# ha7ilm/csdr

Measured on AMD Instinct MI355X. Metric: complex MS/s in->out, WFM demod chain @2.4 MS/s x N streams, higher is better.
Workload: dtype f32

## Files before the change

### csdr_amd/csrc/wfm_mfma.hip

```cpp
#include "common.hpp"
#include "wfm_mfma.hpp"
#include <hip/hip_ext.h>
#include <math.h>
#include <string.h>
#include <stdlib.h>
#include <complex>
#include <vector>
using namespace csdr_amd;

namespace csdr_amd {

bool wfm_mfma_supported(int D, int L, int F)
{
    if ((D * F) & 1) return false;
    const int win_off = (18 * D) & ~15;
    const int span_bytes = 2 * (D * (3 * F + 10) + L) - win_off;
    if (span_bytes > 64 * WFM_NK) return false;
    if (D + L + 3 * D * F + 8 > WFM_HIST) return false;
    return true;
}

void wfm_mfma_build_table(int D, int L, int F, float shift_rate, const float *taps, WfmMfmaTable &t)
{
    t.D = D; t.L = L; t.F = F;
// ... 21 lines not shown
            const int q = r / 4, which = (r % 4) / 2, comp = r % 2;
            const long off = (long)D * (F * q + 9 + which) - base_off_samples;
            for (int tp = 0; tp < L; tp++) {
                const long ts = off + tp;
                const std::complex<double> G = a * (double)taps[tp] * std::polar(pow(mag, (double)ts), ang * (double)ts);
                for (int c = 0; c < 2; c++) {
                    const double val = comp == 0 ? (c == 0 ? G.real() : -G.imag()) : (c == 0 ? G.imag() : G.real());
                    const long colb = 2 * ts + c;
                    const int ks = (int)(colb / 64), b = (int)(colb % 64);
                    long qv = lrint(val * qs);
                    const int w2 = (int)(((qv + 128) % 256 + 256) % 256) - 128; qv = (qv - w2) / 256;
                    const int w1 = (int)(((qv + 128) % 256 + 256) % 256) - 128; qv = (qv - w1) / 256;
                    const int dig[3] = {(int)qv, w1, w2};
                    for (int l = 0; l < 3; l++) t.seq_frags[((size_t)(ks * 3 + l) * 64 + (16 * (b / 16) + r)) * 16 + b % 16] = (int8_t)dig[l];
                    gsum[(size_t)(colb / 16) * 16 + r] += val;
                }
            }
        }
        t.seq_cum.assign((size_t)(ngr + 1) * 16, 0.f);
        for (int r = 0; r < 16; r++) {
            double run = 0;
            for (int g = 0; g <= ngr; g++) { t.seq_cum[(size_t)g * 16 + r] = (float)(0.5 * run); if (g < ngr) run += gsum[(size_t)g * 16 + r]; }
        }
    }
}

}

namespace {

typedef int v4i __attribute__((ext_vector_type(4)));

__device__ __forceinline__ float combine_digits(int a0, int a1, int a2)
{
    return fmaf((float)a0, 65536.0f, fmaf((float)a1, 256.0f, (float)a2));
}

__device__ __forceinline__ void tile_rows(const v4i (&acc)[3], const v4i (&snap)[3], bool two, float scale, const float (&k0)[4], const float (&k1)[4],
                                          float2 C0, float2 C1, float &pI, float &pQ, float &cI, float &cQ)
{
    float u0[4];
    if (two) {
        float u1[4];
#pragma unroll
        for (int r = 0; r < 4; r++) {
            u0[r] = fmaf(combine_digits(snap[0][r], snap[1][r], snap[2][r]), scale, k0[r]);
            u1[r] = fmaf(combine_digits(acc[0][r] - snap[0][r], acc[1][r] - snap[1][r], acc[2][r] - snap[2][r]), scale, k1[r]);
        }
        pI = C0.x * u0[0] - C0.y * u0[1] + (C1.x * u1[0] - C1.y * u1[1]); pQ = C0.x * u0[1] + C0.y * u0[0] + (C1.x * u1[1] + C1.y * u1[0]);
        cI = C0.x * u0[2] - C0.y * u0[3] + (C1.x * u1[2] - C1.y * u1[3]); cQ = C0.x * u0[3] + C0.y * u0[2] + (C1.x * u1[3] + C1.y * u1[2]);
    } else {
#pragma unroll
        for (int r = 0; r < 4; r++) u0[r] = fmaf(combine_digits(acc[0][r], acc[1][r], acc[2][r]), scale, k0[r]);
        pI = C0.x * u0[0] - C0.y * u0[1]; pQ = C0.x * u0[1] + C0.y * u0[0];
        cI = C0.x * u0[2] - C0.y * u0[3]; cQ = C0.x * u0[3] + C0.y * u0[2];
    }
}

template <int N> __device__ __forceinline__ void wait_vmcnt() { asm volatile("s_waitcnt vmcnt(%0)" :: "n"(N) : "memory"); }

template <int KB>
__device__ __forceinline__ void wfm_chain(const v4i (&A)[WFM_NK * 3], const v4i (&Bf)[WFM_NK], bool lo_lane, v4i (&acc)[3], v4i (&snap)[3])
{
    const v4i z = {0, 0, 0, 0};
#pragma unroll
    for (int ks = 0; ks < WFM_NK; ks++) {
        if (ks == KB) {
            const v4i lo = lo_lane ? Bf[ks] : z, hi = lo_lane ? z : Bf[ks];
#pragma unroll
            for (int l = 0; l < 3; l++) acc[l] = __builtin_amdgcn_mfma_i32_16x16x64_i8(A[ks * 3 + l], lo, acc[l], 0, 0, 0);
#pragma unroll
            for (int l = 0; l < 3; l++) snap[l] = acc[l];
#pragma unroll
            for (int l = 0; l < 3; l++) acc[l] = __builtin_amdgcn_mfma_i32_16x16x64_i8(A[ks * 3 + l], hi, acc[l], 0, 0, 0);
        } else {
#pragma unroll
            for (int l = 0; l < 3; l++) acc[l] = __builtin_amdgcn_mfma_i32_16x16x64_i8(A[ks * 3 + l], Bf[ks], acc[l], 0, 0, 0);
        }
    }
}

struct SeqParams {
    int n_streams; long long B2; long long tile_first; int n_tiles, tiles_per_seg;
    int stride, win_off; float scale;
    long long two_T;
    float alpha; const float *last_in; float *last_out; int16_t *s16; float *af; size_t out_pitch; long long j_first; int n_audio;
    const uint8_t *head_in; uint8_t *head_out;
    long long col_bytes; int col_chunks, col_audio, n_cols;
    size_t frag_stride, tab_pitch; int tab_len;
    const float *scales;
    const float *lead_d; const int *lead_n; int lead_stride;
};

#ifndef SEQ_RB_KIB
#define SEQ_RB_KIB 9
#endif
constexpr int SEQ_RB = 1024 * SEQ_RB_KIB;
#ifndef SEQ_RING_PAD
#define SEQ_RING_PAD 32
#endif
constexpr int SEQ_RP = SEQ_RB + SEQ_RING_PAD;
constexpr int SEQ_NGR = 4 * WFM_NK;
#ifndef SEQ_TPG_N
#define SEQ_TPG_N 6
#endif
#ifndef SEQ_NLD_N
#define SEQ_NLD_N 2
#endif
constexpr int SEQ_TPG = SEQ_TPG_N;
constexpr int SEQ_NLD = SEQ_NLD_N;
constexpr int SEQ_NW = SEQ_TPG + SEQ_NLD;
constexpr int SEQ_NLW = SEQ_NLD;
constexpr int SEQ_LINE = 64;
constexpr int SEQ_OUTS = (SEQ_LINE - 1 + 3 * 4 * SEQ_TPG + 4 * SEQ_TPG - 1) / (4 * SEQ_TPG);
constexpr int SEQ_OUTR = SEQ_OUTS * 4 * SEQ_TPG;
constexpr int SEQ_OUTP = SEQ_OUTR + 4;
static_assert(16 % SEQ_NLW == 0 && (16 / SEQ_NLW) * 7 <= 63 && SEQ_TPG % 2 == 0, "rows per fetching wave (vmcnt counts to 63); the de-emphasis scan works on pairs");
constexpr int SEQ_HEAD = 1024;

#ifndef WFM_DIAG
#define WFM_DIAG 0
#endif
#ifdef WFM_PROF
__device__ unsigned long long g_wfm_prof[SEQ_NW][8];
__device__ unsigned long long g_wfm_life[SEQ_NW][4];
#define PROF_T(k) { const long long t_now = __builtin_readcyclecounter(); prof[k] += t_now - t_prev; t_prev = t_now; }
#else
#define PROF_T(k)
#endif

constexpr int RES_WARM = 48;
struct ResCtl {
    const uint32_t *desc;
    const uint32_t *ctrl;
    uint32_t *done;
    unsigned *cnt;
    unsigned long long *t_first;
    unsigned long long *next_item;
    unsigned *exiting;
    const uint8_t *in_ring; int16_t *out_ring; size_t in_slot_bytes, out_slot_elems;
    int n_slots, desc_lines, n_wsb, T, D, L, F;
    long long idle_ticks, life_ticks;
    const float *lead_d; int lead_stride;
    const float *lead_state;
    unsigned long long *stats;
    int fence_mode;
};
__device__ __forceinline__ uint32_t sys_load(const uint32_t *p) { return __hip_atomic_load(p, __ATOMIC_RELAXED, __HIP_MEMORY_SCOPE_SYSTEM); }
__device__ __forceinline__ uint32_t res_tag(long long k) { return (uint32_t)((unsigned long long)k % 0xfffffffeull) + 1u; }

template <bool PS, bool RES = false>
__global__ __launch_bounds__(64 * SEQ_NW) void k_wfm_mfma_seq(const uint8_t *__restrict__ in, size_t in_pitch, const v4i *__restrict__ frags, const float *__restrict__ cum,
                                                               const float2 *__restrict__ dtab, const float2 *__restrict__ ctab, SeqParams p_in, ResCtl rc)
{
    static_assert(!(PS && RES), "the resident form exists for the shared-rate kernel");
    constexpr int TPG = SEQ_TPG, SPW = 16 / SEQ_NLW, NTHR = 64 * SEQ_NW;
    extern __shared__ float4 lds_raw[];
    uint8_t *lds_in = reinterpret_cast<uint8_t *>(lds_raw);
    float *lds_out = reinterpret_cast<float *>(lds_in + 16 * SEQ_RP);
    float *lcum = lds_out + 16 * SEQ_OUTP;
    float2 *ctl = reinterpret_cast<float2 *>(lcum + (SEQ_NGR + 1) * 16);
    const int tid = threadIdx.x, wv = __builtin_amdgcn_readfirstlane(tid >> 6), lane = tid & 63, col = lane & 15, q = lane >> 4;
    const bool fetches = wv >= TPG;
#ifdef WFM_PROF
    const long long t_entry = __builtin_readcyclecounter();
    long long t_first = t_entry, t_last = t_entry;
#endif
    const int fw = wv - TPG;
    float scale = p_in.scale;
    if constexpr (PS) { const int sbp = blockIdx.x; frags += (size_t)sbp * p_in.frag_stride; cum += (size_t)sbp * ((SEQ_NGR + 1) * 16); dtab += (size_t)sbp * 3072; ctab += sbp; scale = p_in.scales[sbp]; }
    for (int i = tid; i < (SEQ_NGR + 1) * 16; i += NTHR) lcum[i] = cum[i];
    v4i A[WFM_NK * 3];
#pragma unroll
    for (int s = 0; s < WFM_NK * 3; s++) A[s] = frags[s * 64 + lane];

    float c_lo[4], c_hi[4];
    {
        const float4 a = *reinterpret_cast<const float4 *>(cum + 4 * q), b = *reinterpret_cast<const float4 *>(cum + (size_t)SEQ_NGR * 16 + 4 * q);
        c_lo[0] = a.x; c_lo[1] = a.y; c_lo[2] = a.z; c_lo[3] = a.w; c_hi[0] = b.x; c_hi[1] = b.y; c_hi[2] = b.z; c_hi[3] = b.w;
    }
    const float K = 0.340447550238101026565118445432744920253753662109375f;
    SeqParams p_res;
    if constexpr (RES) p_res = p_in;
    const SeqParams &p = RES ? p_res : p_in;
    unsigned long long item = 0;
    long long res_t_launch = 0;
    uint32_t *const rctl = reinterpret_cast<uint32_t *>(ctl);
    const float2 *const lseed = ctl + 1;
    long long st_wait = 0, st_body = 0, st_done = 0, st_items = 0, st_t = 0;
    if constexpr (RES) { item = rc.next_item[blockIdx.x]; res_t_launch = wall_clock64(); st_t = res_t_launch; }
    bool pend = false; unsigned pend_c = 0; int pend_slot = 0, pend_n = 0; long long pend_k = 0;
    uint32_t pre_v[4] = {0u, 0u, 0u, 0u}; bool pre_valid = false;
    auto res_complete = [&]() {
        if constexpr (RES) {
            if (tid == 0 && pend) {
                pend = false;
                if (pend_c + 1 == (unsigned)rc.n_wsb) {
                    const unsigned long long tf = __hip_atomic_exchange(rc.t_first + pend_slot, ~0ull, __ATOMIC_RELAXED, __HIP_MEMORY_SCOPE_AGENT), td = (unsigned long long)wall_clock64();
                    __hip_atomic_store(rc.cnt + pend_slot, 0u, __ATOMIC_RELAXED, __HIP_MEMORY_SCOPE_AGENT);
                    uint32_t *dn = rc.done + (size_t)pend_slot * 16;
                    __hip_atomic_store(dn + 1, (uint32_t)pend_n, __ATOMIC_RELAXED, __HIP_MEMORY_SCOPE_SYSTEM);
                    __hip_atomic_store(dn + 2, (uint32_t)tf, __ATOMIC_RELAXED, __HIP_MEMORY_SCOPE_SYSTEM); __hip_atomic_store(dn + 3, (uint32_t)(tf >> 32), __ATOMIC_RELAXED, __HIP_MEMORY_SCOPE_SYSTEM);
                    __hip_atomic_store(dn + 4, (uint32_t)td, __ATOMIC_RELAXED, __HIP_MEMORY_SCOPE_SYSTEM); __hip_atomic_store(dn + 5, (uint32_t)(td >> 32), __ATOMIC_RELAXED, __HIP_MEMORY_SCOPE_SYSTEM);
                    asm volatile("s_waitcnt vmcnt(0)" ::: "memory");
                    __hip_atomic_store(dn, res_tag(pend_k), __ATOMIC_RELAXED, __HIP_MEMORY_SCOPE_SYSTEM);
                }
            }
        }
    };
    for (;;) {
    int res_slot = 0, res_lead = 0; long long res_k = 0; bool res_retuned = false;
    const uint8_t *pblock = nullptr;
    if constexpr (RES) {
        res_k = (long long)(item / (unsigned)rc.n_wsb);
        res_slot = (int)(res_k % rc.n_slots);
        if (wv == 0) {
            const uint32_t *dsc = rc.desc + (size_t)res_slot * rc.desc_lines * 16;
            const uint32_t tag = res_tag(res_k);
            const int nd = rc.desc_lines * 16;
            const long long t_wait = wall_clock64();
            uint32_t state = 0;
            for (int iter = 0;; iter++) {
                uint32_t v[4] = {0u, 0u, 0u, 0u};
                bool have = false;
                if (iter == 0 && pre_valid) {
#pragma unroll
                    for (int j = 0; j < 4; j++) v[j] = pre_v[j];
                    have = true;
                } else {
                    const uint32_t t0 = sys_load(dsc);
                    if (t0 == tag) {
#pragma unroll
                        for (int j = 0; j < 4; j++) { const int d = lane + 64 * j; v[j] = d < nd ? sys_load(dsc + d) : 0u; }
                        have = true;
                    }
                }
                const uint32_t ex = __hip_atomic_load(rc.exiting, __ATOMIC_RELAXED, __HIP_MEMORY_SCOPE_AGENT);
                const uint32_t stop = (iter & 7) == 7 ? sys_load(rc.ctrl) : 0u;
                res_complete();
                bool ok = have;
#pragma unroll
                for (int j = 0; j < 4; j++) { const int d = lane + 64 * j; if (d < nd && (d & 15) == 0 && v[j] != tag) ok = false; }
                const bool ready = __all(ok);
                const long long now = wall_clock64();
                const bool old = now - res_t_launch > rc.life_ticks;
                if (ready && !ex && !old) {
#pragma unroll
                    for (int j = 0; j < 4; j++) {
                        const int d = lane + 64 * j, w = d & 15;
                        if (d < nd && w >= 2) rctl[2 + (d >> 4) * 14 + (w - 2)] = v[j];
                        if (d == 1) rctl[1] = v[j];
                    }
                    state = 1; break;
                }
                if (ex || old || stop || now - t_wait > rc.idle_ticks) { state = 2; break; }
                if (iter < 2) __builtin_amdgcn_s_sleep(24); else if (iter < 6) __builtin_amdgcn_s_sleep(64); else { __builtin_amdgcn_s_sleep(127); __builtin_amdgcn_s_sleep(100); }
            }
            pre_valid = false;
            if (lane == 0) rctl[0] = state;
        }
        __syncthreads();
        if (rctl[0] != 1u) {
            if (tid == 0) {
                __hip_atomic_store(rc.exiting, 1u, __ATOMIC_RELAXED, __HIP_MEMORY_SCOPE_AGENT); rc.next_item[blockIdx.x] = item;
                unsigned long long *sp = rc.stats + (size_t)blockIdx.x * 4;
                sp[0] += (unsigned long long)st_wait; sp[1] += (unsigned long long)st_body; sp[2] += (unsigned long long)st_done; sp[3] += (unsigned long long)st_items;
            }
            return;
        }
        if (tid == 0) { const long long t = wall_clock64(); st_wait += t - st_t; st_t = t; }
        res_lead = (int)(rctl[1] & 0xffu); res_retuned = (rctl[1] >> 8) & 1u;
        auto j_hi = [&](long long kk) -> long long {
            if (kk < 0) return -1;
            const long long avail_last = (kk + 1) * rc.T - 1;
            if (avail_last - (rc.L - 1) < 0) return -1;
            const long long k_max = (avail_last - (rc.L - 1)) / rc.D;
            return k_max >= 10 ? (k_max - 10) / rc.F : -1;
        };
        const long long jp = j_hi(res_k - 1), jn = j_hi(res_k);
        p_res.B2 = 2 * res_k * rc.T;
        p_res.j_first = jp + 1; p_res.n_audio = (int)(jn - jp);
        p_res.tile_first = p_res.j_first / 4; p_res.n_tiles = (int)((p_res.j_first + p_res.n_audio - 1) / 4 - p_res.tile_first + 1);
        p_res.tiles_per_seg = p_res.n_tiles;
        p_res.s16 = rc.out_ring + (size_t)res_slot * rc.out_slot_elems;
        if (tid == 0) (void)__hip_atomic_fetch_min(rc.t_first + res_slot, (unsigned long long)wall_clock64(), __ATOMIC_RELAXED, __HIP_MEMORY_SCOPE_AGENT);
    }
    const int sb = RES ? (int)(item % (unsigned)rc.n_wsb) : (int)blockIdx.x;
    const int seg_y = RES ? 0 : (int)blockIdx.y;
    const int col0 = PS ? 16 * seg_y : 0;
    if constexpr (RES) {
        in = rc.in_ring + (size_t)res_slot * rc.in_slot_bytes;
        pblock = rc.in_ring + (size_t)((res_slot + rc.n_slots - 1) % rc.n_slots) * rc.in_slot_bytes + (long long)sb * 16 * (long long)in_pitch;
    }
    const long long t0 = p.tile_first + (long long)seg_y * p.tiles_per_seg * (PS ? 16 : 1);
    long long t1 = t0 + p.tiles_per_seg; if (t1 > p.tile_first + p.n_tiles) t1 = p.tile_first + p.n_tiles;
    if (!RES && t0 >= t1) return;
    const int n_it = (int)(t1 - t0), n_grp = (n_it + TPG - 1) / TPG;
    const int n_lead = RES ? res_lead : ((PS && p.lead_n && seg_y == 0) ? p.lead_n[sb] : 0);
    const int n_warm = RES ? ((res_k > 0 && !res_retuned) ? 2 : 0) : ((PS || seg_y > 0) ? 2 : 0);
    const int last_stream = p.n_streams - 1;
    const int tstride = p.stride;
    const long long org = PS ? (long long)col0 * p.col_bytes : 0LL;
    long long wg = (t0 - (long long)n_warm * TPG) * tstride + p.win_off - p.B2 - org;
    const long long F0 = wg & ~1023LL;
    long long F_end = ((t1 - 1) * tstride + p.win_off - p.B2 - org + 64 * WFM_NK + 1023) & ~1023LL;
    { const long long row_end = ((p.two_T + 1023) & ~1023LL) - org; if (F_end > row_end) F_end = row_end; }
    long long F = F0;
    int fslot = (int)((F0 + 2 * SEQ_RB) % SEQ_RB), wslot = (int)((wg + 2 * SEQ_RB) % SEQ_RB);
    const uint32_t lds_in_addr = (uint32_t)(size_t)(__attribute__((address_space(3))) uint8_t *)lds_in;
    uint32_t voff[SPW], voff_h[SPW];
    long long row_lim[SPW];
#pragma unroll
    for (int r = 0; r < SPW; r++) {
        if constexpr (PS) {
            voff[r] = (uint32_t)((long long)(SPW * fw + r) * p.col_bytes) + 16u * lane;
            voff_h[r] = 16u * lane;
            row_lim[r] = p.two_T - (long long)(col0 + SPW * fw + r) * p.col_bytes;
        } else {
            const int srow = max(min(sb * 16 + SPW * fw + r, last_stream) - sb * 16, 0);
            voff[r] = (uint32_t)srow * (uint32_t)in_pitch + 16u * lane;
            voff_h[r] = (uint32_t)srow * (uint32_t)SEQ_HEAD + 16u * lane;
            row_lim[r] = 0;
        }
    }
    const uint8_t *sblock = PS ? in + (long long)sb * (long long)in_pitch + org : in + (long long)sb * 16 * (long long)in_pitch;
    const uint8_t *hblock = PS ? p.head_in + (size_t)sb * SEQ_HEAD : p.head_in + (size_t)sb * 16 * SEQ_HEAD;
    const bool ragged = (p.two_T & 1023) != 0;
    auto row_step = [&]() {
        if constexpr (PS) {
            const uint32_t ldst = lds_in_addr + (SPW * fw) * SEQ_RP + (uint32_t)fslot;
            const bool head = F < 0 && col0 == 0;
            if (!head && !ragged) {
                uint32_t vo[SPW];
#pragma unroll
                for (int r = 0; r < SPW; r++) vo[r] = F < row_lim[r] ? voff[r] : 16u * lane;
                dma_rows<SPW, SEQ_RP>(vo, sblock + F, __builtin_amdgcn_readfirstlane((int)ldst));
            } else
#pragma unroll
            for (int r = 0; r < SPW; r++) {
                const bool hrow = head && (SPW * fw + r == 0 || F + 1024 > row_lim[r]);
                const bool beyond = !hrow && F >= row_lim[r];
                const uint8_t *sbase = hrow ? hblock : sblock + F;
                const uint32_t vo = hrow ? voff_h[r] : (beyond ? 16u * lane : voff[r]);
                const bool live = hrow || F + 16 * lane < (beyond ? p.two_T - org : row_lim[r]);
                const uint32_t la = __builtin_amdgcn_readfirstlane((int)(ldst + r * SEQ_RP));
                uint32_t keep;
                if (live)
                    asm volatile("s_mov_b32 %0, m0\n\ts_mov_b32 m0, %3\n\ts_nop 0\n\tglobal_load_lds_dwordx4 %1, %2 nt\n\ts_mov_b32 m0, %0"
                                 : "=&s"(keep) : "v"(vo), "s"(sbase), "s"(la) : "memory");
            }
            F += 1024; fslot += 1024; if (fslot >= SEQ_RB) fslot -= SEQ_RB;
            return;
        }
        if constexpr (RES) {
            const uint8_t *sb_res = F < 0 ? pblock + (p.two_T + F) : sblock + F;
            dma_rows<SPW, SEQ_RP>(voff, sb_res, __builtin_amdgcn_readfirstlane((int)(lds_in_addr + (SPW * fw) * SEQ_RP + (uint32_t)fslot)));
            F += 1024; fslot += 1024; if (fslot >= SEQ_RB) fslot -= SEQ_RB;
            return;
        }
        const bool head = F < 0;
        const uint8_t *sbase = head ? hblock : sblock + F;
        const uint32_t ldst = lds_in_addr + (SPW * fw) * SEQ_RP + (uint32_t)fslot;
        const bool mask = ragged && !head;
        const bool live = !mask || F + 16 * lane < p.two_T;
        if (!head && !ragged) dma_rows<SPW, SEQ_RP>(voff, sbase, __builtin_amdgcn_readfirstlane((int)ldst));
        else
#pragma unroll
        for (int r = 0; r < SPW; r++) {
            const uint32_t la = __builtin_amdgcn_readfirstlane((int)(ldst + r * SEQ_RP));
            const uint32_t vo = head ? voff_h[r] : voff[r];
            uint32_t keep;
            if (!mask)
                asm volatile("s_mov_b32 %0, m0\n\ts_mov_b32 m0, %3\n\ts_nop 0\n\tglobal_load_lds_dwordx4 %1, %2 nt\n\ts_mov_b32 m0, %0"
                             : "=&s"(keep) : "v"(vo), "s"(sbase), "s"(la) : "memory");
            else if (live)
                asm volatile("s_mov_b32 %0, m0\n\ts_mov_b32 m0, %3\n\ts_nop 0\n\tglobal_load_lds_dwordx4 %1, %2 nt\n\ts_mov_b32 m0, %0"
                             : "=&s"(keep) : "v"(vo), "s"(sbase), "s"(la) : "memory");
        }
// ... 395 lines not shown
    const int s = blockIdx.x, t = threadIdx.x;
    for (int k = 2 * t; k < 2 * t + 2; k++) {
        const long long pos = two_T - 512 + k;
        head_out[(size_t)s * SEQ_HEAD + 512 + k] = pos >= 0 ? in[(size_t)s * in_pitch + pos] : head_in[(size_t)s * SEQ_HEAD + 512 + (pos + 512)];
    }
}

struct LeadParams { int D, L, F; long long B, j_first, c_first; int n_lead, ja0, lead_stride; float *warm; size_t tab_pitch, dtab_stride, ct_stride, head_pitch, head_off; };
__global__ __launch_bounds__(128) void k_wfm_lead(const uint8_t *__restrict__ in, size_t in_pitch, const uint8_t *__restrict__ head, const float *__restrict__ taps,
                                                 const float2 *__restrict__ ctab, const float2 *__restrict__ dtab, const float2 *__restrict__ dtab_old,
                                                 const int *__restrict__ list, float *__restrict__ lead_d, LeadParams p)
{
    __shared__ float2 yv[2];
    const int s = list[blockIdx.y], ja = (int)blockIdx.x + p.ja0, which = threadIdx.x >> 6, lane = threadIdx.x & 63;
    const long long j = p.j_first + ja, k = (long long)p.F * j + 9 + which;
    const uint8_t *row = in + (size_t)s * in_pitch, *hrow = head + (size_t)s * p.head_pitch + p.head_off;
    const float2 *ct = ctab + (size_t)s * p.ct_stride, *dn = dtab + (size_t)s * p.dtab_stride, *dold = dtab_old + (size_t)s * p.dtab_stride;
    float ai = 0.f, aq = 0.f;
    for (int t = lane; t < p.L; t += 64) {
        const long long n = (long long)p.D * k + t, rel = n - p.B;
        uint32_t vi, vq;
        if (rel < 0) { vi = hrow[2 * (rel + 256)]; vq = hrow[2 * (rel + 256) + 1]; } else { vi = row[2 * rel]; vq = row[2 * rel + 1]; }
        const float2 C = ct[(size_t)((n >> 10) - p.c_first) * p.tab_pitch], Dv = (rel < 0 ? dold : dn)[(int)(n & 1023) + 2048];
        const float2 R = make_float2(C.x * Dv.x - C.y * Dv.y, C.x * Dv.y + C.y * Dv.x);
        const float xi = fmaf((float)vi, 0x1.010102p-7f, -1.0f), xq = fmaf((float)vq, 0x1.010102p-7f, -1.0f);
        const float h = taps[t];
        ai = fmaf(h, xi * R.x - xq * R.y, ai); aq = fmaf(h, xq * R.x + xi * R.y, aq);
    }
#pragma unroll
    for (int o = 32; o >= 1; o >>= 1) { ai += __shfl_xor(ai, o, 64); aq += __shfl_xor(aq, o, 64); }
    if (lane == 0) yv[which] = make_float2(ai, aq);
    __syncthreads();
    if (threadIdx.x == 0) {
        const float K = 0.340447550238101026565118445432744920253753662109375f;
        const float pI = yv[0].x, pQ = yv[0].y, cI = yv[1].x, cQ = yv[1].y;
        const float dq = cQ - pQ, di = cI - pI, num = cI * dq - cQ * di, den = cI * cI + cQ * cQ;
        float rd = __builtin_amdgcn_rcpf(den); rd = fmaf(fmaf(-den, rd, 1.0f), rd, rd);
        const float dv = (den != 0.f) ? (K * num) * rd : 0.f;
        if (ja >= 0) lead_d[(size_t)s * p.lead_stride + ja] = dv; else p.warm[(size_t)s * RES_WARM + (ja + RES_WARM)] = dv;
    }
}

__global__ __launch_bounds__(64) void k_wfm_lead_state(const float *__restrict__ warm, float *__restrict__ state, int n_streams, float alpha)
{
    const int s = blockIdx.x * 64 + threadIdx.x;
    if (s >= n_streams) return;
    float y = 0.f;
    for (int i = 0; i < RES_WARM; i++) y = alpha * warm[(size_t)s * RES_WARM + i] + (1 - alpha) * y;
    state[s] = y;
}

}

namespace csdr_amd {

size_t wfm_mfma_head_bytes(int n_streams) { return (size_t)((n_streams + 15) / 16 * 16) * SEQ_HEAD; }

int wfm_mfma_lead(hipStream_t st, const uint8_t *in, size_t in_pitch, const uint8_t *head, const float *d_taps, const float2 *ctab, size_t tab_pitch, const float2 *d_dtab,
                  const float2 *d_dtab_old, const int *d_list, int n_list, float *d_lead_d, int lead_stride, int D, int L, int F, long long B, long long j_first, int n_lead)
{
    if (n_list <= 0 || n_lead <= 0) return 0;
    LeadParams lp; lp.D = D; lp.L = L; lp.F = F; lp.B = B; lp.j_first = j_first; lp.n_lead = n_lead; lp.tab_pitch = tab_pitch; lp.dtab_stride = 3072;
    lp.ct_stride = 1; lp.head_pitch = SEQ_HEAD; lp.head_off = 512; lp.c_first = (B >> 10) - 1; lp.ja0 = 0; lp.warm = nullptr; lp.lead_stride = lead_stride;
    hipLaunchKernelGGL(k_wfm_lead, dim3(n_lead, n_list), dim3(128), 0, st, in, in_pitch, head, d_taps, ctab, d_dtab, d_dtab_old, d_list, d_lead_d, lp);
    CSDR_LAUNCH_CHECK();
    return 0;
}

int wfm_mfma_lead_shared(hipStream_t st, const uint8_t *in, size_t in_pitch, const uint8_t *prev, size_t two_T, const float *d_taps, const float2 *ctab, const float2 *d_dtab,
                         const float2 *d_dtab_old, const int *d_list, int n_list, float *d_lead_d, int lead_stride, float *d_warm, float *d_state, float alpha,
                         int D, int L, int F, long long B, long long j_first, int n_lead)
{
    if (n_list <= 0) return 0;
    if (j_first < RES_WARM) return fail_msg(-3, "wfm ring: a retune needs %d audio samples in front of the block", RES_WARM);
    LeadParams lp; lp.D = D; lp.L = L; lp.F = F; lp.B = B; lp.j_first = j_first; lp.n_lead = n_lead; lp.tab_pitch = 1; lp.dtab_stride = 0;
    lp.ct_stride = 0; lp.head_pitch = in_pitch; lp.head_off = two_T - 512; lp.c_first = (B >> 10) - 4; lp.ja0 = -RES_WARM; lp.warm = d_warm; lp.lead_stride = lead_stride;
    hipLaunchKernelGGL(k_wfm_lead, dim3(n_lead + RES_WARM, n_list), dim3(128), 0, st, in, in_pitch, prev, d_taps, ctab, d_dtab, d_dtab_old, d_list, d_lead_d, lp);
    CSDR_LAUNCH_CHECK();
    hipLaunchKernelGGL(k_wfm_lead_state, dim3((n_list + 63) / 64), dim3(64), 0, st, d_warm, d_state, n_list, alpha);
    CSDR_LAUNCH_CHECK();
    return 0;
}

int wfm_mfma_launch(hipStream_t st, hipEvent_t ev_begin, hipEvent_t ev_end, const uint8_t *in, size_t in_pitch, const WfmMfmaDevice &dev, const float2 *ctab,
                    int n_streams, int T, long long B, long long j_first, int n_audio, const WfmBackArgs &back, const WfmPerStream *ps)
{
    if (in_pitch * 16 + 4096 >= ((size_t)1 << 32)) return fail_msg(-3, "wfm: in_pitch %zu too large for the matrix-core front end (32-bit row offsets)", in_pitch);
    if (n_audio <= 0) {
        hipLaunchKernelGGL(k_wfm_roll_head, dim3(n_streams), dim3(256), 0, st, in, in_pitch, 2LL * T, back.head_in, back.head_out);
        CSDR_LAUNCH_CHECK();
        return 0;
    }
    SeqParams sp;
    memset((void *)&sp, 0, sizeof sp);
    ResCtl no_res; memset((void *)&no_res, 0, sizeof no_res);
    sp.n_streams = n_streams; sp.B2 = 2 * B; sp.two_T = 2LL * T;
    sp.tile_first = j_first / 4; sp.n_tiles = (int)((j_first + n_audio - 1) / 4 - sp.tile_first + 1);
    sp.stride = dev.tile_stride_bytes; sp.win_off = dev.win_off_bytes; sp.scale = dev.seq_scale;
    const int n_cu = current_device_cu_count();
    const int n_wsb = (n_streams + 15) / 16;
    int n_seg = (n_cu + n_wsb - 1) / n_wsb; if (n_seg < 1) n_seg = 1;
    if (n_seg > sp.n_tiles / 24) n_seg = sp.n_tiles / 24;
    if (n_seg < 1) n_seg = 1;
    sp.tiles_per_seg = ((sp.n_tiles + n_seg - 1) / n_seg + SEQ_TPG - 1) / SEQ_TPG * SEQ_TPG;
    n_seg = (sp.n_tiles + sp.tiles_per_seg - 1) / sp.tiles_per_seg;
    sp.alpha = back.alpha; sp.last_in = back.last_in; sp.last_out = back.last_out; sp.s16 = back.s16; sp.af = back.af; sp.out_pitch = back.out_pitch;
    sp.j_first = j_first; sp.n_audio = n_audio; sp.head_in = back.head_in; sp.head_out = back.head_out;
    if (ps) {
        const long long ts = sp.stride / 2;
        long long per = ts; { long long a = per, b = 1024; while (b) { const long long t = a % b; a = b; b = t; } per = per / a * 1024; }
        int tpp = (int)(per / ts);
        while ((4 * tpp) % SEQ_LINE) tpp *= 2;
        const int n_per = (sp.n_tiles + tpp - 1) / tpp;
        int n_ss = (4 * n_cu + n_streams - 1) / n_streams; if (n_ss < 1) n_ss = 1;
        int np = (n_per + 16 * n_ss - 1) / (16 * n_ss); if (np < 1) np = 1;
        sp.tiles_per_seg = np * tpp;
        sp.n_cols = (sp.n_tiles + sp.tiles_per_seg - 1) / sp.tiles_per_seg;
        n_seg = (sp.n_cols + 15) / 16;
        sp.col_bytes = (long long)sp.tiles_per_seg * sp.stride; sp.col_chunks = (int)(sp.col_bytes / 2048); sp.col_audio = 4 * sp.tiles_per_seg;
        sp.frag_stride = (size_t)WFM_NK * 3 * 64; sp.tab_pitch = ps->tab_pitch; sp.tab_len = ps->tab_len; sp.scales = ps->d_scales;
        sp.lead_d = ps->d_lead_d; sp.lead_n = ps->d_lead_n; sp.lead_stride = ps->lead_stride;
        if (sp.col_bytes * 16 + 4096 >= (1LL << 32)) return fail_msg(-3, "wfm: block too large for the per-stream kernel's 32-bit row offsets");
        const size_t ldsp = (size_t)16 * SEQ_RP + 16 * SEQ_OUTP * sizeof(float) + (SEQ_NGR + 1) * 16 * sizeof(float) + 2 * 48 * sizeof(float2);
        { const int arc = lds_attr_once((const void *)k_wfm_mfma_seq<true>, ldsp); if (arc) return arc; }
        if (ev_begin && ev_end)
            hipExtLaunchKernelGGL(k_wfm_mfma_seq<true>, dim3(n_streams, n_seg), dim3(64 * SEQ_NW), ldsp, st, ev_begin, ev_end, 0, in, in_pitch, (const v4i *)dev.d_seq_frags, dev.d_seq_cum, dev.d_dtab, ctab, sp, no_res);
        else
            hipLaunchKernelGGL(k_wfm_mfma_seq<true>, dim3(n_streams, n_seg), dim3(64 * SEQ_NW), ldsp, st, in, in_pitch, (const v4i *)dev.d_seq_frags, dev.d_seq_cum, dev.d_dtab, ctab, sp, no_res);
        CSDR_LAUNCH_CHECK();
        if (T < 256 || (T & 7)) {
            hipLaunchKernelGGL(k_wfm_roll_head, dim3(n_streams), dim3(256), 0, st, in, in_pitch, 2LL * T, back.head_in, back.head_out);
            CSDR_LAUNCH_CHECK();
        }
        return 0;
    }
    const size_t lds = (size_t)16 * SEQ_RP + 16 * SEQ_OUTP * sizeof(float) + (SEQ_NGR + 1) * 16 * sizeof(float);
    { const int arc = lds_attr_once((const void *)k_wfm_mfma_seq<false>, lds); if (arc) return arc; }
    if (ev_begin && ev_end)
        hipExtLaunchKernelGGL(k_wfm_mfma_seq<false>, dim3(n_wsb, n_seg), dim3(64 * SEQ_NW), lds, st, ev_begin, ev_end, 0, in, in_pitch, (const v4i *)dev.d_seq_frags, dev.d_seq_cum, dev.d_dtab, ctab, sp, no_res);
    else
        hipLaunchKernelGGL(k_wfm_mfma_seq<false>, dim3(n_wsb, n_seg), dim3(64 * SEQ_NW), lds, st, in, in_pitch, (const v4i *)dev.d_seq_frags, dev.d_seq_cum, dev.d_dtab, ctab, sp, no_res);
    CSDR_LAUNCH_CHECK();
    if (T < 256 || (T & 7)) {
        hipLaunchKernelGGL(k_wfm_roll_head, dim3(n_streams), dim3(256), 0, st, in, in_pitch, 2LL * T, back.head_in, back.head_out);
        CSDR_LAUNCH_CHECK();
    }
    return 0;
}

int wfm_mfma_launch_resident(hipStream_t st, hipEvent_t ev_end, const WfmMfmaDevice &dev, int n_streams, size_t in_pitch, float alpha, size_t out_pitch, const WfmResident &rv, int grid)
{
    if (in_pitch * 16 + 4096 >= ((size_t)1 << 32)) return fail_msg(-3, "wfm ring: in_pitch %zu too large (32-bit row offsets)", in_pitch);
    SeqParams sp; memset((void *)&sp, 0, sizeof sp);
    sp.n_streams = n_streams; sp.two_T = 2LL * rv.T; sp.stride = dev.tile_stride_bytes; sp.win_off = dev.win_off_bytes; sp.scale = dev.seq_scale;
    sp.alpha = alpha; sp.out_pitch = out_pitch;
    ResCtl rc; memset((void *)&rc, 0, sizeof rc);
    rc.desc = rv.desc; rc.ctrl = rv.ctrl; rc.done = rv.done; rc.cnt = rv.cnt; rc.t_first = rv.t_first; rc.next_item = rv.next_item; rc.exiting = rv.exiting;
    rc.in_ring = rv.in_ring; rc.out_ring = rv.out_ring; rc.in_slot_bytes = rv.in_slot_bytes; rc.out_slot_elems = rv.out_slot_elems;
    rc.n_slots = rv.n_slots; rc.desc_lines = rv.desc_lines; rc.n_wsb = (n_streams + 15) / 16; rc.T = rv.T; rc.D = rv.D; rc.L = rv.L; rc.F = rv.F;
    rc.idle_ticks = rv.idle_ticks; rc.life_ticks = rv.life_ticks; rc.lead_d = rv.lead_d; rc.lead_stride = rv.lead_stride; rc.lead_state = rv.lead_state; rc.stats = rv.stats; rc.fence_mode = rv.fence_mode;
    if (rv.desc_lines < 1 || rv.desc_lines > 16) return fail_msg(-3, "wfm ring: %d descriptor lines", rv.desc_lines);
    const size_t lds = (size_t)16 * SEQ_RP + 16 * SEQ_OUTP * sizeof(float) + (SEQ_NGR + 1) * 16 * sizeof(float) + 8 + (size_t)rv.desc_lines * 14 * sizeof(float);
    { const int arc = lds_attr_once((const void *)k_wfm_mfma_seq<false, true>, lds); if (arc) return arc; }
    hipLaunchKernelGGL((k_wfm_mfma_seq<false, true>), dim3(grid), dim3(64 * SEQ_NW), lds, st, (const uint8_t *)nullptr, in_pitch, (const v4i *)dev.d_seq_frags, dev.d_seq_cum, dev.d_dtab,
                       (const float2 *)nullptr, sp, rc);
    CSDR_LAUNCH_CHECK();
    if (ev_end) CSDR_HIP(hipEventRecord(ev_end, st));
    return 0;
}
int wfm_resident_max_grid() { return current_device_cu_count(); }

}

#ifdef WFM_PROF
extern "C" int csdr_amd_debug_wfm_prof(unsigned long long *out, int reset)
{
    if (hipMemcpyFromSymbol(out, HIP_SYMBOL(g_wfm_prof), sizeof(unsigned long long) * SEQ_NW * 8) != hipSuccess) return -1;
    if (reset) { static unsigned long long z[SEQ_NW * 8]; if (hipMemcpyToSymbol(HIP_SYMBOL(g_wfm_prof), z, sizeof(z)) != hipSuccess) return -1; }
    return 0;
}
extern "C" int csdr_amd_debug_wfm_life(unsigned long long *out, int reset)
{
    if (hipMemcpyFromSymbol(out, HIP_SYMBOL(g_wfm_life), sizeof(unsigned long long) * SEQ_NW * 4) != hipSuccess) return -1;
    if (reset) { static unsigned long long z[SEQ_NW * 4]; if (hipMemcpyToSymbol(HIP_SYMBOL(g_wfm_life), z, sizeof(z)) != hipSuccess) return -1; }
    return 0;
}
#endif

extern "C" int csdr_amd_debug_wfm_seq_tile(int D, int L, int F, float shift_rate, const float *taps, long long n0, const uint8_t *window,
                                           const float *ctab2, float *out16)
{
    if (!wfm_mfma_supported(D, L, F) || (n0 & 7)) return -1;
    static WfmMfmaTable t; static int cD = 0, cL = 0, cF = 0; static float crate = 0; static std::vector<float> ctaps;
    if (cD != D || cL != L || cF != F || crate != shift_rate || ctaps != std::vector<float>(taps, taps + L)) {
        wfm_mfma_build_table(D, L, F, shift_rate, taps, t); cD = D; cL = L; cF = F; crate = shift_rate; ctaps.assign(taps, taps + L);
    }
    const int off = (int)(n0 & 1023);
    const bool two = off + 32 * WFM_NK > 1024;
    const int bo = 2 * (1024 - off), kb = two ? (bo >> 6) : WFM_NK, hq = (bo >> 4) & 3, gb = bo >> 4;
    const float2 D0 = t.dtab[off + 2048], C0 = make_float2(ctab2[0], ctab2[1]);
    const float2 P0 = make_float2(C0.x * D0.x - C0.y * D0.y, C0.x * D0.y + C0.y * D0.x);
    float2 P1 = make_float2(0.f, 0.f);
    if (two) { const float2 D1 = t.dtab[off - 1024 + 2048], C1 = make_float2(ctab2[2], ctab2[3]); P1 = make_float2(C1.x * D1.x - C1.y * D1.y, C1.x * D1.y + C1.y * D1.x); }
    const int ngr = 4 * WFM_NK;
    float u[16], v[16];
    for (int r = 0; r < 16; r++) {
        long acc[3] = {0, 0, 0}, snap[3] = {0, 0, 0};
        auto step = [&](int ks, int kg_lo, int kg_hi) {
            for (int kg = kg_lo; kg < kg_hi; kg++) for (int b = 0; b < 16; b++) {
                const int x = (int)(int8_t)(window[64 * ks + 16 * kg + b] ^ 0x80);
                for (int l = 0; l < 3; l++) acc[l] += (long)t.seq_frags[((size_t)(ks * 3 + l) * 64 + (16 * kg + r)) * 16 + b] * x;
            }
        };
        for (int ks = 0; ks < WFM_NK; ks++) {
            if (ks == kb) { step(ks, 0, hq); for (int l = 0; l < 3; l++) snap[l] = acc[l]; step(ks, hq, 4); }
            else step(ks, 0, 4);
        }
        const float clo = t.seq_cum[r], chi = t.seq_cum[(size_t)ngr * 16 + r];
        if (two) {
            const float cb = t.seq_cum[(size_t)gb * 16 + r];
            u[r] = fmaf(fmaf((float)snap[0], 65536.0f, fmaf((float)snap[1], 256.0f, (float)snap[2])), t.seq_scale, cb - clo);
            v[r] = fmaf(fmaf((float)(acc[0] - snap[0]), 65536.0f, fmaf((float)(acc[1] - snap[1]), 256.0f, (float)(acc[2] - snap[2]))), t.seq_scale, chi - cb);
        } else {
            u[r] = fmaf(fmaf((float)acc[0], 65536.0f, fmaf((float)acc[1], 256.0f, (float)acc[2])), t.seq_scale, chi - clo);
            v[r] = 0.f;
        }
    }
    for (int k = 0; k < 8; k++) {
        out16[2 * k] = P0.x * u[2 * k] - P0.y * u[2 * k + 1] + (P1.x * v[2 * k] - P1.y * v[2 * k + 1]);
        out16[2 * k + 1] = P0.x * u[2 * k + 1] + P0.y * u[2 * k] + (P1.x * v[2 * k + 1] + P1.y * v[2 * k]);
    }
    return 0;
}
```

### csdr_amd/csrc/wfm_mfma.hpp

```cpp
#pragma once
#include "common.hpp"
#include <vector>

namespace csdr_amd {

constexpr int WFM_HIST = 256;
constexpr int WFM_NK = 8;

struct WfmMfmaTable {
    int D, L, F, tile_stride_bytes, win_off_bytes;
    std::vector<int8_t> seq_frags;
    std::vector<float> seq_cum;
    std::vector<float2> dtab;
    float seq_scale;
};

struct WfmMfmaDevice {
    int tile_stride_bytes, win_off_bytes;
    void *d_seq_frags; float *d_seq_cum; float2 *d_dtab; float seq_scale;
};

struct WfmBackArgs {
    float alpha; const float *last_in; float *last_out; int16_t *s16; float *af; size_t out_pitch; const uint8_t *head_in; uint8_t *head_out;
};

struct WfmPerStream { size_t tab_pitch; int tab_len; const float *d_scales; const float *d_lead_d; const int *d_lead_n; int lead_stride; };
inline int wfm_lead_max(int D, int L, int F) { return (D + L - 1) / (D * F) + 2; }

struct WfmResident {
    const uint32_t *desc, *ctrl; uint32_t *done;
    unsigned *cnt; unsigned long long *t_first, *next_item; unsigned *exiting;
    const uint8_t *in_ring; int16_t *out_ring; size_t in_slot_bytes, out_slot_elems;
    int n_slots, desc_lines, T, D, L, F;
    long long idle_ticks, life_ticks;
    const float *lead_d, *lead_state; int lead_stride;
    unsigned long long *stats; int fence_mode;
};
constexpr int WFM_RES_WARM = 48;
int wfm_mfma_launch_resident(hipStream_t st, hipEvent_t ev_end, const WfmMfmaDevice &dev, int n_streams, size_t in_pitch, float alpha, size_t out_pitch, const WfmResident &rv, int grid);
int wfm_resident_max_grid();
int wfm_mfma_lead_shared(hipStream_t st, const uint8_t *in, size_t in_pitch, const uint8_t *prev, size_t two_T, const float *d_taps, const float2 *ctab, const float2 *d_dtab,
                         const float2 *d_dtab_old, const int *d_list, int n_list, float *d_lead_d, int lead_stride, float *d_warm, float *d_state, float alpha,
                         int D, int L, int F, long long B, long long j_first, int n_lead);

bool wfm_mfma_supported(int D, int L, int F);
void wfm_mfma_build_table(int D, int L, int F, float shift_rate, const float *taps, WfmMfmaTable &t);
size_t wfm_mfma_head_bytes(int n_streams);
int wfm_mfma_launch(hipStream_t st, hipEvent_t ev_begin, hipEvent_t ev_end, const uint8_t *in, size_t in_pitch, const WfmMfmaDevice &dev, const float2 *ctab,
                    int n_streams, int T, long long B, long long j_first, int n_audio, const WfmBackArgs &back, const WfmPerStream *ps = nullptr);
int wfm_mfma_lead(hipStream_t st, const uint8_t *in, size_t in_pitch, const uint8_t *head, const float *d_taps, const float2 *ctab, size_t tab_pitch, const float2 *d_dtab,
                  const float2 *d_dtab_old, const int *d_list, int n_list, float *d_lead_d, int lead_stride, int D, int L, int F, long long B, long long j_first, int n_lead);

}
```

### include/csdr_amd.h

```cpp
#ifndef CSDR_AMD_H
#define CSDR_AMD_H
#include <stddef.h>
#include <stdint.h>

#ifdef __cplusplus
extern "C" {
#endif

typedef struct csdr_complexf_s { float i, q; } csdr_complexf;

typedef enum { CSDR_WINDOW_BOXCAR = 0, CSDR_WINDOW_BLACKMAN = 1, CSDR_WINDOW_HAMMING = 2 } csdr_window_t;

typedef struct csdr_amd_ctx csdr_amd_ctx;

csdr_amd_ctx *csdr_amd_ctx_create(int device, void *hip_stream);
void          csdr_amd_ctx_destroy(csdr_amd_ctx *ctx);
int           csdr_amd_ctx_sync(csdr_amd_ctx *ctx);
void         *csdr_amd_ctx_stream(csdr_amd_ctx *ctx);
const char   *csdr_amd_last_error(void);
int           csdr_amd_device_count(void);
const char   *csdr_amd_device_arch(csdr_amd_ctx *ctx);

void *csdr_amd_malloc(csdr_amd_ctx *ctx, size_t bytes);
void  csdr_amd_free(csdr_amd_ctx *ctx, void *dptr);
// ... 531 lines not shown
int  csdr_amd_wfm_ring_set_rate(csdr_amd_wfm_ring *r, float shift_rate);
float csdr_amd_wfm_ring_get_rate(const csdr_amd_wfm_ring *r);
int  csdr_amd_wfm_ring_set_timeouts(csdr_amd_wfm_ring *r, double idle_us, double life_ms);
int  csdr_amd_wfm_ring_resident(csdr_amd_wfm_ring *r);
int  csdr_amd_wfm_ring_stop(csdr_amd_wfm_ring *r);
int  csdr_amd_wfm_ring_slots(const csdr_amd_wfm_ring *r);
int  csdr_amd_wfm_ring_grid(const csdr_amd_wfm_ring *r);
long csdr_amd_wfm_ring_launches(const csdr_amd_wfm_ring *r);
long long csdr_amd_wfm_ring_submitted(const csdr_amd_wfm_ring *r);
int  csdr_amd_wfm_ring_stats(csdr_amd_wfm_ring *r, double out[4]);
int  csdr_amd_wfm_ring_replay(csdr_amd_wfm_ring *r, long n_blocks, double *t_first_us, double *t_done_us);
int  csdr_amd_wfm_ring_block_times(csdr_amd_wfm_ring *r, long long seq, double *t_first_us, double *t_done_us);

typedef struct csdr_amd_ddc csdr_amd_ddc;
csdr_amd_ddc *csdr_amd_ddc_create(csdr_amd_ctx *ctx, int n_streams, float shift_rate, int decimation,
                                  const float *host_taps, int taps_length, size_t max_block_samples);
csdr_amd_ddc *csdr_amd_ddc_create_rates(csdr_amd_ctx *ctx, int n_streams, const float *shift_rates, int decimation,
                                        const float *host_taps, int taps_length, size_t max_block_samples);
int   csdr_amd_ddc_set_rate(csdr_amd_ddc *d, int stream, float shift_rate);
float csdr_amd_ddc_get_rate(const csdr_amd_ddc *d, int stream);
int   csdr_amd_ddc_fallback(const csdr_amd_ddc *d);
void csdr_amd_ddc_destroy(csdr_amd_ddc *d);
int  csdr_amd_ddc_reset(csdr_amd_ddc *d);
long csdr_amd_ddc_process(csdr_amd_ddc *d, const uint8_t *in, size_t in_pitch, size_t block_samples,
                          csdr_complexf *out, size_t out_pitch);
const char *csdr_amd_ddc_kernel_name(const csdr_amd_ddc *d);
int csdr_amd_ddc_set_profiling(csdr_amd_ddc *d, int on);
int csdr_amd_ddc_kernel_time(csdr_amd_ddc *d, double *total_ms, long *launches);
int csdr_amd_debug_ddc_mfma_tile(int D, int L, float shift_rate, const float *taps, long long n0, const uint8_t *window,
                                 const float *ctab3, float *out16);

typedef struct csdr_amd_nfm csdr_amd_nfm;
csdr_amd_nfm *csdr_amd_nfm_create(csdr_amd_ctx *ctx, int n_streams, float shift_rate, int decimation, const float *host_taps, int taps_length,
                                  int audio_rate, int agc_block, float agc_reference, float limit_max, size_t max_block_samples);
csdr_amd_nfm *csdr_amd_nfm_create_rates(csdr_amd_ctx *ctx, int n_streams, const float *shift_rates, int decimation, const float *host_taps, int taps_length,
                                        int audio_rate, int agc_block, float agc_reference, float limit_max, size_t max_block_samples);
int  csdr_amd_nfm_set_rate(csdr_amd_nfm *w, int stream, float shift_rate);
void csdr_amd_nfm_destroy(csdr_amd_nfm *w);
int  csdr_amd_nfm_reset(csdr_amd_nfm *w);
long csdr_amd_nfm_process(csdr_amd_nfm *w, const uint8_t *in, size_t in_pitch, size_t block_samples,
                          int16_t *audio_s16, float *audio_f, size_t out_pitch);
csdr_amd_ddc *csdr_amd_nfm_front_end(csdr_amd_nfm *w);

enum { CSDR_AMD_AMSSB_AM = 0, CSDR_AMD_AMSSB_SSB = 1 };
typedef struct csdr_amd_amssb_params {
    int mode, block;
    float reference, attack_rate, decay_rate, max_gain;
    short hang_time, attack_wait_time;
    float gain_filter_alpha, limit_max;
} csdr_amd_amssb_params;
typedef struct csdr_amd_amssb_chan { float last_dc, last_gain; } csdr_amd_amssb_chan;
typedef struct csdr_amd_amssb csdr_amd_amssb;
int  csdr_amd_amssb_params_default(csdr_amd_amssb_params *p, int mode);
csdr_amd_amssb *csdr_amd_amssb_create_cf32(csdr_amd_ctx *ctx, const csdr_amd_amssb_params *params, int n_channels, const csdr_complexf *taps, int taps_length,
                                           int fft_size, size_t max_samples_per_call);
csdr_amd_amssb *csdr_amd_amssb_create(csdr_amd_ctx *ctx, const csdr_amd_amssb_params *params, int n_channels, float shift_rate, int decimation,
                                      const float *ddc_taps, int ddc_taps_length, const csdr_complexf *taps, int taps_length, int fft_size,
                                      size_t max_samples_per_call);
csdr_amd_amssb *csdr_amd_amssb_create_rates(csdr_amd_ctx *ctx, const csdr_amd_amssb_params *params, int n_channels, const float *shift_rates, int decimation,
                                            const float *ddc_taps, int ddc_taps_length, const csdr_complexf *taps, int taps_length, int fft_size,
                                            size_t max_samples_per_call);
long long csdr_amd_amssb_process(csdr_amd_amssb *p, const void *in, size_t in_pitch, long long n_in, int16_t *audio_s16, float *pre_agc_f, size_t out_pitch);
long long csdr_amd_amssb_max_out(const csdr_amd_amssb *p, long long n_in);
int  csdr_amd_amssb_set_rate(csdr_amd_amssb *p, int channel, float shift_rate);
float csdr_amd_amssb_get_rate(const csdr_amd_amssb *p, int channel);
csdr_amd_ddc *csdr_amd_amssb_front_end(csdr_amd_amssb *p);
int  csdr_amd_amssb_set_passband(csdr_amd_amssb *p, int channel, float low, float high, int window);
int  csdr_amd_amssb_set_channel_taps(csdr_amd_amssb *p, int channel, const csdr_complexf *taps, int taps_length);
int  csdr_amd_amssb_get_passband(const csdr_amd_amssb *p, int channel, float *low, float *high);
int  csdr_amd_amssb_reset(csdr_amd_amssb *p);
int  csdr_amd_amssb_reset_channel(csdr_amd_amssb *p, int channel);
int  csdr_amd_amssb_get_channel(csdr_amd_amssb *p, int channel, csdr_amd_amssb_chan *out);
int  csdr_amd_amssb_set_channel(csdr_amd_amssb *p, int channel, const csdr_amd_amssb_chan *state);
int  csdr_amd_amssb_set_lanes(csdr_amd_amssb *p, int lanes);
int  csdr_amd_amssb_lanes(const csdr_amd_amssb *p);
int  csdr_amd_amssb_force_generic(csdr_amd_amssb *p, int on);
const char *csdr_amd_amssb_kernel_name(const csdr_amd_amssb *p);
void csdr_amd_amssb_destroy(csdr_amd_amssb *p);
long long csdr_amd_debug_amssb_walk(const csdr_amd_amssb_params *params, const csdr_complexf *in, int n_blocks, csdr_amd_amssb_chan *state_io, int16_t *s16_out,
                                    float *pre_agc_out);

int csdr_amd_debug_wfm_seq_tile(int D, int L, int F, float shift_rate, const float *taps, long long n0, const uint8_t *window,
                                const float *ctab2, float *out16);
void csdr_amd_debug_dft16(const float *in32, float *out32, int inverse);
int  csdr_amd_debug_fftfilt_lds(int n, const float *taps_iq, int taps_len, const float *x_iq, long m_new, float *y_iq);
void csdr_amd_debug_dft8(const float *in16, float *out16, int inverse);
int  csdr_amd_debug_ddc_chain(int mode, float rate2, int post_in, int post_dec, int n_blocks, int *remain_io, float *phase_io, float *phases_out, int *count_out);
int  csdr_amd_debug_ddc_fold_plan(int pre_decimation, int n_blocks, int *tiles, long *lds_bytes);
int csdr_amd_debug_nfm_deemph_tile(int audio_rate, float max_amp, const float *x, float *out16);
int csdr_amd_debug_waterfall_row(int fft_size, int every_n_samples, int window, int avgnumber, float add_db, int in_format, const void *in, long long n_in,
                                 float *db_row, float *power_row);
#ifdef __cplusplus
}
#endif
#endif
```

Measured before the change: 2.915 million.

## Balance WFM segment split by giving the first segment the warm-up tiles

Replaces the inline segment-count heuristic with a planner that gives the first segment extra tiles. Later segments must re-run two groups of warm-up tiles, which the first segment skips, so the extra tiles even out per-segment work and shorten the critical path across CUs. The prologue is also changed so fetch-only waves skip loading MFMA fragments and the prefix table, and the table copy is done in two fixed rounds instead of a strided loop. The planner can choose fewer segments than before, which lowers parallelism on short blocks.

```diff
diff --git a/csdr_amd/csrc/wfm_mfma.hip b/csdr_amd/csrc/wfm_mfma.hip
--- a/csdr_amd/csrc/wfm_mfma.hip
+++ b/csdr_amd/csrc/wfm_mfma.hip
@@ -127,6 +127,7 @@
 
 struct SeqParams {
     int n_streams; long long B2; long long tile_first; int n_tiles, tiles_per_seg;
+    int first_extra;
     int stride, win_off; float scale;
     long long two_T;
     float alpha; const float *last_in; float *last_out; int16_t *s16; float *af; size_t out_pitch; long long j_first; int n_audio;
@@ -199,7 +200,7 @@
                                                                const float2 *__restrict__ dtab, const float2 *__restrict__ ctab, SeqParams p_in, ResCtl rc)
 {
     static_assert(!(PS && RES), "the resident form exists for the shared-rate kernel");
-    constexpr int TPG = SEQ_TPG, SPW = 16 / SEQ_NLW, NTHR = 64 * SEQ_NW;
+    constexpr int TPG = SEQ_TPG, SPW = 16 / SEQ_NLW;
     extern __shared__ float4 lds_raw[];
     uint8_t *lds_in = reinterpret_cast<uint8_t *>(lds_raw);
     float *lds_out = reinterpret_cast<float *>(lds_in + 16 * SEQ_RP);
@@ -214,14 +215,19 @@
     const int fw = wv - TPG;
     float scale = p_in.scale;
     if constexpr (PS) { const int sbp = blockIdx.x; frags += (size_t)sbp * p_in.frag_stride; cum += (size_t)sbp * ((SEQ_NGR + 1) * 16); dtab += (size_t)sbp * 3072; ctab += sbp; scale = p_in.scales[sbp]; }
-    for (int i = tid; i < (SEQ_NGR + 1) * 16; i += NTHR) lcum[i] = cum[i];
+    constexpr bool tables_by_all = RES;
+    static_assert(!RES || 64 * SEQ_NW <= (SEQ_NGR + 1) * 16, "every thread copies the prefix table entry of its own index");
     v4i A[WFM_NK * 3];
-#pragma unroll
-    for (int s = 0; s < WFM_NK * 3; s++) A[s] = frags[s * 64 + lane];
-
     float c_lo[4], c_hi[4];
-    {
+    if (tables_by_all || !fetches) {
+        constexpr int NCUM = (SEQ_NGR + 1) * 16, NCT = 64 * TPG;
+        static_assert(NCUM >= NCT && NCUM <= 2 * NCT, "the prefix table is copied in two rounds");
+        const int i1 = min(tid + NCT, NCUM - 1);
+        const float u0 = cum[tid], u1 = cum[i1];
+#pragma unroll
+        for (int s = 0; s < WFM_NK * 3; s++) A[s] = frags[s * 64 + lane];
         const float4 a = *reinterpret_cast<const float4 *>(cum + 4 * q), b = *reinterpret_cast<const float4 *>(cum + (size_t)SEQ_NGR * 16 + 4 * q);
+        lcum[tid] = u0; lcum[i1] = u1;
         c_lo[0] = a.x; c_lo[1] = a.y; c_lo[2] = a.z; c_lo[3] = a.w; c_hi[0] = b.x; c_hi[1] = b.y; c_hi[2] = b.z; c_hi[3] = b.w;
     }
     const float K = 0.340447550238101026565118445432744920253753662109375f;
@@ -337,8 +343,8 @@
         in = rc.in_ring + (size_t)res_slot * rc.in_slot_bytes;
         pblock = rc.in_ring + (size_t)((res_slot + rc.n_slots - 1) % rc.n_slots) * rc.in_slot_bytes + (long long)sb * 16 * (long long)in_pitch;
     }
-    const long long t0 = p.tile_first + (long long)seg_y * p.tiles_per_seg * (PS ? 16 : 1);
-    long long t1 = t0 + p.tiles_per_seg; if (t1 > p.tile_first + p.n_tiles) t1 = p.tile_first + p.n_tiles;
+    const long long t0 = p.tile_first + (long long)seg_y * p.tiles_per_seg * (PS ? 16 : 1) + (seg_y > 0 ? p.first_extra : 0);
+    long long t1 = t0 + p.tiles_per_seg + (seg_y > 0 ? 0 : p.first_extra); if (t1 > p.tile_first + p.n_tiles) t1 = p.tile_first + p.n_tiles;
     if (!RES && t0 >= t1) return;
     const int n_it = (int)(t1 - t0), n_grp = (n_it + TPG - 1) / TPG;
     const int n_lead = RES ? res_lead : ((PS && p.lead_n && seg_y == 0) ? p.lead_n[sb] : 0);
@@ -900,6 +906,23 @@
     return 0;
 }
 
+int wfm_segment_plan(int n_tiles, int n_wsb, int n_cu, int *n_seg, int *tiles_per_seg, int *first_extra)
+{
+    if (n_tiles < 1 || n_wsb < 1 || n_cu < 1) return -1;
+    const int warm = 2 * SEQ_TPG;
+    const long long max_seg = ((long long)n_cu + n_wsb - 1) / n_wsb;
+    const int steps_one = (n_tiles + SEQ_TPG - 1) / SEQ_TPG;
+    *n_seg = 1; *tiles_per_seg = steps_one * SEQ_TPG; *first_extra = 0;
+    if (max_seg < 2 || n_tiles <= 2 * warm) return 0;
+    const long long rest = n_tiles - warm;
+    long long tps = ((rest + max_seg - 1) / max_seg + SEQ_TPG - 1) / SEQ_TPG * SEQ_TPG;
+    if (tps < warm) tps = warm;
+    const long long k = (rest + tps - 1) / tps;
+    if (k < 2 || tps / SEQ_TPG + 2 >= steps_one) return 0;
+    *n_seg = (int)k; *tiles_per_seg = (int)tps; *first_extra = warm;
+    return 0;
+}
+
 int wfm_mfma_launch(hipStream_t st, hipEvent_t ev_begin, hipEvent_t ev_end, const uint8_t *in, size_t in_pitch, const WfmMfmaDevice &dev, const float2 *ctab,
                     int n_streams, int T, long long B, long long j_first, int n_audio, const WfmBackArgs &back, const WfmPerStream *ps)
 {
@@ -917,11 +940,8 @@
     sp.stride = dev.tile_stride_bytes; sp.win_off = dev.win_off_bytes; sp.scale = dev.seq_scale;
     const int n_cu = current_device_cu_count();
     const int n_wsb = (n_streams + 15) / 16;
-    int n_seg = (n_cu + n_wsb - 1) / n_wsb; if (n_seg < 1) n_seg = 1;
-    if (n_seg > sp.n_tiles / 24) n_seg = sp.n_tiles / 24;
-    if (n_seg < 1) n_seg = 1;
-    sp.tiles_per_seg = ((sp.n_tiles + n_seg - 1) / n_seg + SEQ_TPG - 1) / SEQ_TPG * SEQ_TPG;
-    n_seg = (sp.n_tiles + sp.tiles_per_seg - 1) / sp.tiles_per_seg;
+    int n_seg = 1;
+    wfm_segment_plan(sp.n_tiles, n_wsb, n_cu, &n_seg, &sp.tiles_per_seg, &sp.first_extra);
     sp.alpha = back.alpha; sp.last_in = back.last_in; sp.last_out = back.last_out; sp.s16 = back.s16; sp.af = back.af; sp.out_pitch = back.out_pitch;
     sp.j_first = j_first; sp.n_audio = n_audio; sp.head_in = back.head_in; sp.head_out = back.head_out;
     if (ps) {
@@ -932,7 +952,7 @@
         const int n_per = (sp.n_tiles + tpp - 1) / tpp;
         int n_ss = (4 * n_cu + n_streams - 1) / n_streams; if (n_ss < 1) n_ss = 1;
         int np = (n_per + 16 * n_ss - 1) / (16 * n_ss); if (np < 1) np = 1;
-        sp.tiles_per_seg = np * tpp;
+        sp.tiles_per_seg = np * tpp; sp.first_extra = 0;
         sp.n_cols = (sp.n_tiles + sp.tiles_per_seg - 1) / sp.tiles_per_seg;
         n_seg = (sp.n_cols + 15) / 16;
         sp.col_bytes = (long long)sp.tiles_per_seg * sp.stride; sp.col_chunks = (int)(sp.col_bytes / 2048); sp.col_audio = 4 * sp.tiles_per_seg;
@@ -1005,6 +1025,11 @@
 }
 #endif
 
+extern "C" int csdr_amd_debug_wfm_segments(int n_tiles, int n_wsb, int n_cu, int *n_seg, int *tiles_per_seg, int *first_extra)
+{
+    return wfm_segment_plan(n_tiles, n_wsb, n_cu, n_seg, tiles_per_seg, first_extra);
+}
+
 extern "C" int csdr_amd_debug_wfm_seq_tile(int D, int L, int F, float shift_rate, const float *taps, long long n0, const uint8_t *window,
                                            const float *ctab2, float *out16)
 {
diff --git a/csdr_amd/csrc/wfm_mfma.hpp b/csdr_amd/csrc/wfm_mfma.hpp
--- a/csdr_amd/csrc/wfm_mfma.hpp
+++ b/csdr_amd/csrc/wfm_mfma.hpp
@@ -46,6 +46,7 @@
 bool wfm_mfma_supported(int D, int L, int F);
 void wfm_mfma_build_table(int D, int L, int F, float shift_rate, const float *taps, WfmMfmaTable &t);
 size_t wfm_mfma_head_bytes(int n_streams);
+int wfm_segment_plan(int n_tiles, int n_wsb, int n_cu, int *n_seg, int *tiles_per_seg, int *first_extra);
 int wfm_mfma_launch(hipStream_t st, hipEvent_t ev_begin, hipEvent_t ev_end, const uint8_t *in, size_t in_pitch, const WfmMfmaDevice &dev, const float2 *ctab,
                     int n_streams, int T, long long B, long long j_first, int n_audio, const WfmBackArgs &back, const WfmPerStream *ps = nullptr);
 int wfm_mfma_lead(hipStream_t st, const uint8_t *in, size_t in_pitch, const uint8_t *head, const float *d_taps, const float2 *ctab, size_t tab_pitch, const float2 *d_dtab,
diff --git a/include/csdr_amd.h b/include/csdr_amd.h
--- a/include/csdr_amd.h
+++ b/include/csdr_amd.h
@@ -637,6 +637,7 @@
 
 int csdr_amd_debug_wfm_seq_tile(int D, int L, int F, float shift_rate, const float *taps, long long n0, const uint8_t *window,
                                 const float *ctab2, float *out16);
+int csdr_amd_debug_wfm_segments(int n_tiles, int n_wsb, int n_cu, int *n_seg, int *tiles_per_seg, int *first_extra);
 void csdr_amd_debug_dft16(const float *in32, float *out32, int inverse);
 int  csdr_amd_debug_fftfilt_lds(int n, const float *taps_iq, int taps_len, const float *x_iq, long m_new, float *y_iq);
 void csdr_amd_debug_dft8(const float *in16, float *out16, int inverse);
```

New measurement: 2.913 million. Within noise of the previous version (-0.1%).
